# YuliangXiu/ICON

Measured on AMD Instinct MI355X. Metric: query-points/sec at 256^3 grid, higher is better.
Workload: dtype f32 via 3x f16 split MFMA (22-bit operands, f32 accumulate)

## Files before the change

icon_amd/csrc/fused_f16x3.hip:

```cpp
#pragma clang fp contract(off)

#include "geom_device.h"
#include "batch_device.h"
#include "mlp_f16x3_device.h"
#include "mlp_plain_device.h"
#include "sign_list_device.h"

#include <algorithm>
#include <mutex>

namespace icon {

constexpr int kTilePts = kF16Pts;
constexpr int kXsOff = kSideOff + 4352;
constexpr int kFusedLds = kXsOff + kTilePts * kXRow * 4;

struct FusedGeom {
    MeshDev m;
    FeatDev f;
    Calib cal;
    int res, z0;
    int off, nx, zs;
    const float *pts;
    int64_t N;
    const int *n_dev;
    const int32_t *out_map;
    float sdf_clip;
    int cmap_local;
    NearRef near;
    const uint8_t *code8;
    const int64_t *block_offsets;
    const unsigned long long *grp_mask;
    SignSrc sg;
    unsigned long long *clock;
    unsigned int *steal;
    int steal_static, steal_grp, steal_ngrp;
};
constexpr int kPoolOff = kSideOff + kSideFloats * 4;
enum { kPoolNext = 0, kPoolMask, kPoolDone, kPoolPer, kPoolRem, kPoolStatic, kPoolGroup, kPoolNGrp, kPoolGrid, kPoolWords };
static_assert(kPoolOff + 4 * kPoolWords <= kSideOff + 4352, "the draw state lives in the slack behind the side arrays");
constexpr int kPoolLenShift = 24;
constexpr int kMaxStealGroup = 127;

__device__ __forceinline__ void pool_draw(unsigned int *steal, volatile int *pool)
{
    unsigned xcc;
    asm volatile("s_getreg_b32 %0, hwreg(HW_REG_XCC_ID)" : "=s"(xcc));
    const int per = pool[kPoolPer], rem = pool[kPoolRem], stat = pool[kPoolStatic], grp = pool[kPoolGroup], ngrp = pool[kPoolNGrp],
              grid = pool[kPoolGrid];
    int mask = pool[kPoolMask], word = -1;
    for (int s = 0; s < 8 && word < 0; ++s) {
        const int x = (int)((xcc + (unsigned)s) & 7u);
        if ((mask >> x) & 1) continue;
        const int nwg = (grid - x + 7) >> 3;
        for (;;) {
            const int t = (int)atomicAdd(steal + x, 1u);
            if (t >= nwg * ngrp) { mask |= 1 << x; break; }
            const int k = t / ngrp, g = t - k * ngrp, b = x + 8 * k;
            const int sb = b * per + min(b, rem), eb = sb + per + (b < rem ? 1 : 0);
            const int a = sb + stat + g * grp;
            if (a < eb) { word = a | (min(grp, eb - a) << kPoolLenShift); break; }
        }
    }
    pool[kPoolMask] = mask;
    pool[kPoolNext] = word;
}

__device__ __forceinline__ void wg_stamp(unsigned long long *rec)
{
    rec[0] = __builtin_readcyclecounter();
    rec[1] = __builtin_amdgcn_s_memrealtime();
}

static_assert(kScanBlock == 256, "k_sign's 256-point blocks are the blocks of the outlier scan and the tiles of the fused kernel");
template <bool LATTICE>
// ... 73 lines not shown
        load_tri_full(m.tris + m.bin_slots[k], a, b, c, ia, ib, ic);
        cnt += ray_hit(p, a, b, c, ia, ib, ic);
    }
    cnt += __shfl_xor(cnt, 1);
    cnt += __shfl_xor(cnt, 2);
    if (live) {
        const bool ins = brute ? inside_brute(m, p) : ((cnt & 1) != 0);
        const bool far = box_dist2(d.box_lo[0], d.box_lo[1], d.box_lo[2], d.box_hi[0], d.box_hi[1], d.box_hi[2], p) > far_box2 || near_is_far(near, i);
        code = far ? sign_code_far(p, ins) : sign_code(p, near_d2(near, i), ins, sdf_clip);
        if (s == 0) code8[i] = (uint8_t)code;
    }
    unsigned long long x = __ballot(live && s == 0 && (code & kCodeOutlier));
    x = (x | (x >> 3)) & 0x0303030303030303ull;
    x = (x | (x >> 6)) & 0x000f000f000f000full;
    x = (x | (x >> 12)) & 0x000000ff000000ffull;
    x = (x | (x >> 24)) & 0xffffull;
    const int wave = threadIdx.x >> 6;
    if ((threadIdx.x & 63) == 0 && x) atomicOr(&gm[wave >> 2], x << (16 * (wave & 3)));
    __syncthreads();
    if (threadIdx.x < 4) grp_mask[(int64_t)blockIdx.x * 4 + threadIdx.x] = gm[threadIdx.x];
    if (threadIdx.x == 0) block_counts[blockIdx.x] = __popcll(gm[0]) + __popcll(gm[1]) + __popcll(gm[2]) + __popcll(gm[3]);
}

__global__ __launch_bounds__(256) void k_shell_zero(float *__restrict__ out, int res, int z0, int za, int zb, int row_wgs)
{
    const int planes = zb - za;
    if ((int)blockIdx.x < row_wgs) {
        const int64_t row = (int64_t)blockIdx.x * 256 + threadIdx.x;
        if (row >= (int64_t)planes * res) return;
        const int iy = (int)(row % res), iz = za + (int)(row / res);
        float *o = out + ((int64_t)(iz - z0) * res + iy) * res;
        o[0] = 0.0f; o[res - 1] = 0.0f;
        return;
    }
    const int f = ((int)blockIdx.x - row_wgs) * 4 + (int)(threadIdx.x >> 6);
    const int lane = threadIdx.x & 63;
    int iy, iz;
    if (f < 2 * planes) { iz = za + (f >> 1); iy = (f & 1) ? res - 1 : 0; }
    else {
        const int g = f - 2 * planes;
        const bool has0 = za == 0, has1 = zb == res;
        const int pl = g / res;
        if (pl >= (has0 ? 1 : 0) + (has1 ? 1 : 0)) return;
        iz = (pl == 0 && has0) ? 0 : res - 1;
        iy = g % res;
    }
    float *o = out + ((int64_t)(iz - z0) * res + iy) * res;
    for (int x = lane; x < res; x += 64) o[x] = 0.0f;
}

__device__ __forceinline__ int64_t lattice_item(const FusedGeom &G, int64_t q, int &ix, int &iy, int &iz)
{
    const uint32_t nx = (uint32_t)G.nx, qq = (uint32_t)q;
    const uint32_t r = qq / nx, lx = qq - r * nx, lz = r / nx, ly = r - lz * nx;
    ix = G.off + (int)lx; iy = G.off + (int)ly; iz = G.zs + (int)lz;
    return ((int64_t)(iz - G.z0) * G.res + iy) * G.res + ix;
}

__device__ __forceinline__ int64_t uniform64(int64_t v)
{
    const uint32_t lo = (uint32_t)__builtin_amdgcn_readfirstlane((int)(uint32_t)v);
    const uint32_t hi = (uint32_t)__builtin_amdgcn_readfirstlane((int)(uint32_t)((uint64_t)v >> 32));
    return (int64_t)(((uint64_t)hi << 32) | lo);
}

__device__ __forceinline__ void icon_row(const FusedGeom &G, const MeshDev &m, const FeatDev &f, f3 p, int64_t i, float *xrow, int64_t K, int64_t rank0)
{
    const uint32_t code = G.code8[i];
    Nearest nr;
    nr.slot = near_slot_of(G.near, i); nr.face = 0;
    nr.d2 = (code & kCodeOutlier) ? 0.0f : near_d2(G.near, i);
    const SdfOut o = sdf_attrs(m, p, nr, (code & kCodeInside) != 0);
    float s = o.sdf;
    f3 cmv = o.cm;
    if (code & kCodeOutlier) {
        s = (float)code_sign(code);
        if (G.cmap_local) cmv = mk3(s, s, s);
        else if (K > 0 && (f.smpl_mask & kSmplCmap)) {
            const int64_t blk = i >> 8;
            const int g = (int)(i >> 6) & 3;
            const unsigned long long *mk = G.grp_mask + blk * 4;
            int before = __popcll(mk[g] & ((1ull << (i & 63)) - 1ull));
            if (g > 0) before += __popcll(mk[0]);
            if (g > 1) before += __popcll(mk[1]);
            if (g > 2) before += __popcll(mk[2]);
            const int64_t jr = rank0 + G.block_offsets[blk] + before;
            float c3[3];
            outlier_cmap(G.sg, K, jr, c3);
            cmv = mk3(c3[0], c3[1], c3[2]);
        }
    }
    gather_planes_dyn(f, (f.n_select == 2 && o.vis == 0.0f) ? 1 : 0, p.x, p.y, xrow);
    int hh = f.csel;
    xrow[hh++] = s;
    if (f.smpl_mask & kSmplCmap) { xrow[hh] = cmv.x; xrow[hh + 1] = cmv.y; xrow[hh + 2] = cmv.z; hh += 3; }
    if (f.smpl_mask & kSmplNorm) { xrow[hh] = o.nrm.x; xrow[hh + 1] = o.nrm.y; xrow[hh + 2] = o.nrm.z; }
    xrow[kCodeSlot] = __int_as_float((int)(code & kCodeInCube));
}

template <int PRIOR, Src SRC>
__device__ __forceinline__ void build_row(const FusedGeom &G, const BatchDev &bd, int64_t q, float *xrow, int64_t K, int64_t rank0)
{
    f3 p;
    int64_t i;
    const int64_t b = SRC == Src::Batch ? q / bd.n : 0;
    if (SRC == Src::Lattice) {
        int ix, iy, iz;
// ... 40 lines not shown
    }

    issue_units(w.image, smem + kW0Off, kW0Bytes / 1024, wave0, lane0);
    float *side = reinterpret_cast<float *>(smem + kSideOff);
    for (int i = threadIdx.x; i < kSideFloats; i += kF16Block) side[i] = w.side[i];
    const float *sb0 = side, *sb1 = side + 512, *sb2 = side + 768, *sw3 = side + kW3Float;
    int64_t K = 0, rank0 = 0;
    if (PRIOR == ICON_PRIOR_ICON) launch_sign_extent(G, K, rank0);
    K = uniform64(K); rank0 = uniform64(rank0);

    if (SRC != Src::Batch && G.n_dev) { G.N = *G.n_dev; if (G.N <= 0) return; }
    const int tp = (SMALL && G.N <= (int64_t)(kTilePts / 2) * gridDim.x) ? kTilePts / 2 : kTilePts;
    const int ntiles = (int)((G.N + tp - 1) / tp);
    const bool stealing = !SMALL && G.steal != nullptr;
    const int per = ntiles / (int)gridDim.x, rem = ntiles % (int)gridDim.x;
    int tile = (int)blockIdx.x * per + min((int)blockIdx.x, rem);
    int tile_end = tile + (stealing ? min(G.steal_static, per) : per + ((int)blockIdx.x < rem ? 1 : 0));
    tile = __builtin_amdgcn_readfirstlane(tile);
    tile_end = __builtin_amdgcn_readfirstlane(tile_end);
    volatile int *pool = reinterpret_cast<volatile int *>(smem + kPoolOff);
    if (!SMALL) {
        if (threadIdx.x == 0) {
            pool[kPoolPer] = per; pool[kPoolRem] = rem; pool[kPoolStatic] = G.steal_static; pool[kPoolGroup] = G.steal_grp;
            pool[kPoolNGrp] = G.steal_ngrp; pool[kPoolGrid] = (int)gridDim.x; pool[kPoolDone] = 0; pool[kPoolMask] = 0; pool[kPoolNext] = -1;
            if (stealing && tile >= tile_end) pool_draw(G.steal, pool);
        }
        __syncthreads();
        if (stealing && tile >= tile_end) {
            const int word = __builtin_amdgcn_readfirstlane(pool[kPoolNext]);
            __syncthreads();
            if (word >= 0) { tile = word & ((1 << kPoolLenShift) - 1); tile_end = tile + (word >> kPoolLenShift); }
        }
    }
    if (tile < tile_end) issue_chunk(w.image, smem, 0, wave0, lane0);

    for (int nb = -1; tile < tile_end;) {
        int tid = threadIdx.x;
        asm volatile("" : "+v"(tid));
        const int lane = tid & 63, wave = __builtin_amdgcn_readfirstlane(tid >> 6);
        const int r = lane & 15, g = lane >> 4;
        const int t = tid;
        const bool draw = !SMALL && stealing && tile + 1 == tile_end;
        if (!SMALL && draw && t == 256) pool_draw(G.steal, pool);
        const bool worker = t < tp;
        int64_t q = (int64_t)tile * tp + (worker ? t : 0);
        if (q >= G.N) q = G.N - 1;
        if (worker) build_row<PRIOR, SRC>(G, bd, q, Xs + t * kXRow, K, rank0);
        __syncthreads();

        nb = (!SMALL && draw) ? __builtin_amdgcn_readfirstlane(pool[kPoolNext]) : -1;
        if (!SMALL && tid == 0) pool[kPoolDone] = pool[kPoolDone] + 1;
        const bool more = tile + 1 < tile_end || nb >= 0;
        if (SMALL && wave >= (tp >> 5)) {
            for (int c = 0; c < 16; ++c) {
                issue_chunk(w.image, smem + ((c + 1) & 1) * kBufBytes, c + 1, wave, lane);
                ICON_CHUNK_BARRIER();
            }
            issue_chunk(w.image, smem + kBufBytes, 17, wave, lane);
            ICON_CHUNK_BARRIER();
            issue_chunk(w.image, smem, 18, wave, lane);
            ICON_CHUNK_BARRIER();
            issue_chunk(w.image, smem + kBufBytes, 19, wave, lane);
            ICON_CHUNK_BARRIER();
            if (more) issue_chunk(w.image, smem, 0, wave, lane);
            ++tile;
            continue;
        }
        const int pt = wave * 32 + 16 * (g & 1) + r;
        half8 xb[2];
        const float tail = load_x(Xs + (wave * 32 + r) * kXRow + 8 * (g & 1), Xs + (wave * 32 + 16 + r) * kXRow + 8 * (g & 1), sw3, w.c0, g, xb);
        float maskf = (__float_as_int(Xs[pt * kXRow + kCodeSlot]) & (int)kCodeInCube) ? 1.0f : 0.0f;
        asm volatile("" : "+v"(maskf));

        f32x4 acc1[16][2];
#pragma unroll
        for (int m = 0; m < 16; ++m) acc1[m][0] = acc1[m][1] = *reinterpret_cast<const f32x4 *>(sb1 + m * 16 + 4 * g);
        half8 bh[2], bl[2];
        const LeakyK k0{w.inv0, w.p0, w.q0}, k1{w.inv1, w.p1, w.q1};
        {
            f32x4 h0[2][2];
            l0_tiles(smem + kW0Off, sb0, 0, xb, g, lane, h0);
            activate_split(h0[0][0], h0[0][1], h0[1][0], h0[1][1], k0, bh, bl);
        }
        f32x4 acc2[8][2];
        for (int c = 0; c < 15; ++c) {
            l01_chunk<false>(smem + (c & 1) * kBufBytes, smem + ((c + 1) & 1) * kBufBytes, smem + kW0Off, sb0, w.image, c, acc1, xb,
                             k0, g, lane, wave, bh, bl);
            ICON_CHUNK_BARRIER();
        }
        l01_chunk<true>(smem + kBufBytes, smem, smem + kW0Off, sb0, w.image, 15, acc1, xb, k0, g, lane, wave, bh, bl);
        ICON_CHUNK_BARRIER();
#pragma unroll
        for (int m2 = 0; m2 < 8; ++m2) acc2[m2][0] = acc2[m2][1] = *reinterpret_cast<const f32x4 *>(sb2 + m2 * 16 + 4 * g);
        activate_split(acc1[0][0], acc1[1][0], acc1[0][1], acc1[1][1], k1, bh, bl);
        l2_chunk<0>(smem, smem + kBufBytes, w.image, acc1, acc2, xb, k1, g, lane, wave, bh, bl);
        ICON_CHUNK_BARRIER();
        l2_chunk<1>(smem + kBufBytes, smem, w.image, acc1, acc2, xb, k1, g, lane, wave, bh, bl);
        ICON_CHUNK_BARRIER();
        l2_chunk<2>(smem, smem + kBufBytes, w.image, acc1, acc2, xb, k1, g, lane, wave, bh, bl);
        ICON_CHUNK_BARRIER();
        l2_chunk<3>(smem + kBufBytes, smem, w.image, acc1, acc2, xb, k1, g, lane, wave, bh, bl, more ? 0 : -1);

        float y2[2];
        {
            int tid_3 = threadIdx.x;
            asm volatile("" : "+v"(tid_3), "+v"(acc2[0][0]));
            l3_sum(sw3, acc2, tail, LeakyK{w.inv2, w.p2, w.q2}, w.b3, (tid_3 >> 4) & 3, y2);
        }
        int tid_o = threadIdx.x;
        asm volatile("" : "+v"(tid_o), "+v"(y2[0]), "+v"(y2[1]));
        const int g_o = (tid_o >> 4) & 3, pt_o = (tid_o >> 6) * 32 + 16 * (g_o & 1) + (tid_o & 15);
        const float y = apply_last_op(g_o == 0 ? y2[0] : y2[1], w.last_op);
        const int64_t oq = (int64_t)tile * tp + pt_o;
        if (g_o < 2 && oq < G.N) {
            int ix, iy, iz;
            out[SRC == Src::Lattice ? lattice_item(G, oq, ix, iy, iz) : ((SRC == Src::Points && G.out_map) ? (int64_t)G.out_map[oq] : oq)] = masked_result(y, maskf != 0.0f, w.flag);
        }
        if (!SMALL && nb >= 0) {
            tile = nb & ((1 << kPoolLenShift) - 1);
            tile_end = tile + (nb >> kPoolLenShift);
        } else ++tile;
    }
    if (!SMALL && stealing && threadIdx.x == 0) {
        __threadfence();
        if (atomicAdd(G.steal + 8, 1u) == gridDim.x - 1)
            for (int k = 0; k < 9; ++k) atomicExch(G.steal + k, 0u);
    }
    if (G.clock && threadIdx.x == 0 && blockIdx.x < kMaxProfGrid) {
        if (blockIdx.x == 0) wg_stamp(G.clock + 2);
        unsigned long long *rec = G.clock + 4 + kWgRec * blockIdx.x;
        wg_stamp(rec + 2);
        unsigned xcc, hw;
        asm volatile("s_getreg_b32 %0, hwreg(HW_REG_XCC_ID)" : "=s"(xcc));
        asm volatile("s_getreg_b32 %0, hwreg(HW_REG_HW_ID)" : "=s"(hw));
        rec[4] = ((unsigned long long)xcc << 32) | hw;
        rec[5] = SMALL ? 0ull : (unsigned long long)pool[kPoolDone];
    }
}

template <int PRIOR, Src SRC>
__global__ __launch_bounds__(64) void k_rescue_fused(FusedGeom G, float *__restrict__ out, MlpPlain P, const int *flag, int always, BatchDev bd)
{
    __shared__ float s[kPlainLds];
    if (!always && *flag == 0) return;
    if (SRC != Src::Batch && G.n_dev) G.N = *G.n_dev;
    const int lane = threadIdx.x;
    int64_t K = 0, rank0 = 0;
    if (PRIOR == ICON_PRIOR_ICON) launch_sign_extent(G, K, rank0);
    for (int64_t base = (int64_t)blockIdx.x * 64; base < G.N; base += (int64_t)gridDim.x * 64) {
        const int64_t q = base + lane;
        int ix, iy, iz;
        const int64_t o = q < G.N ? (SRC == Src::Lattice ? lattice_item(G, q, ix, iy, iz) : ((SRC == Src::Points && G.out_map) ? (int64_t)G.out_map[q] : q)) : 0;
        const float v = q < G.N ? out[o] : 0.0f;
        unsigned long long todo = __ballot(not_finite(v));
// ... 41 lines not shown
namespace {
constexpr int kMaxDevices = 64, kMaxKernelIds = 16;
std::mutex g_dev_mutex;
int g_n_cu[kMaxDevices];
bool g_attr_set[kMaxKernelIds][kMaxDevices];
}

int device_cu_count(int *n_cu)
{
    int dev = 0;
    ICON_HIP(hipGetDevice(&dev));
    ICON_ARG(dev >= 0 && dev < kMaxDevices, "device index out of range");
    std::lock_guard<std::mutex> lk(g_dev_mutex);
    if (!g_n_cu[dev]) {
        int n = 0;
        ICON_HIP(hipDeviceGetAttribute(&n, hipDeviceAttributeMultiprocessorCount, dev));
        g_n_cu[dev] = n > 0 ? n : 256;
    }
    *n_cu = g_n_cu[dev];
    return ICON_OK;
}

int once_per_device(int kernel_id, const std::function<hipError_t()> &set)
{
    int dev = 0;
    if (hipGetDevice(&dev) != hipSuccess || dev < 0 || dev >= kMaxDevices || kernel_id < 0 || kernel_id >= kMaxKernelIds) {
        const hipError_t e = set();
        return e == hipSuccess ? ICON_OK : fail(ICON_ERR_HIP, std::string("hipFuncSetAttribute: ") + hipGetErrorString(e));
    }
    std::lock_guard<std::mutex> lk(g_dev_mutex);
    if (g_attr_set[kernel_id][dev]) return ICON_OK;
    const hipError_t e = set();
    if (e != hipSuccess) return fail(ICON_ERR_HIP, std::string("hipFuncSetAttribute: ") + hipGetErrorString(e));
    g_attr_set[kernel_id][dev] = true;
    return ICON_OK;
}

int launch_fused_f16x3(const icon_mesh *mesh, const icon_feat *feat, const icon_mlp *mlp, int prior, const Calib &cal,
                       const LatticeMap &L, int za, int zb, const float *d_points, int64_t N, float sdf_clip, int cmap_local,
                       const icon_work *work, const SignSrc &fs, float *d_occ, bool lattice, hipStream_t st, const BatchDev *bd)
{
    FusedGeom G{};
    if (mesh) G.m = mesh->dev;
    G.f = feat->dev; G.cal = cal; G.pts = d_points; G.sdf_clip = sdf_clip; G.cmap_local = cmap_local;
    if (lattice) {
        const int zs = std::max(za, L.off), ze = std::min(zb, L.res - L.off);
        if (L.off) {
            const int64_t rows = (int64_t)(zb - za) * L.res;
            const int row_wgs = (int)((rows + 255) / 256);
            const int64_t face_rows = 2 * (int64_t)(zb - za) + (int64_t)((za == 0 ? 1 : 0) + (zb == L.res ? 1 : 0)) * L.res;
            if (rows > 0) hipLaunchKernelGGL(k_shell_zero, dim3((unsigned)(row_wgs + (face_rows + 3) / 4)), dim3(256), 0, st, d_occ, L.res, L.z0, za, zb, row_wgs);
        }
        G.res = L.res; G.z0 = L.z0; G.off = L.off; G.nx = L.res - 2 * L.off; G.zs = zs;
        N = (ze > zs) ? (int64_t)(ze - zs) * G.nx * G.nx : 0;
    }
    if (N <= 0) { ICON_HIP(hipGetLastError()); return ICON_OK; }
    ICON_ARG(N < (1ll << 31), "fused: more than 2^31 points in one call");
    G.N = N;
    G.near = work_near(work, mesh); G.code8 = work->d_code8;
    if (!lattice) { G.n_dev = work->q_n_dev; G.out_map = work->q_map; }
    G.clock = work->prof ? work->d_clock : nullptr;
    G.steal = nullptr; G.steal_static = 0; G.steal_grp = 1; G.steal_ngrp = 0;
    G.block_offsets = work->d_block_offsets; G.grp_mask = (const unsigned long long *)work->d_grp_mask;
    G.sg = fs;
    int rc = resolve_signs(work, &G.sg, st);
    if (rc) return rc;
    MlpF16Dev w;
    w.image = mlp->d_f16;
    w.side = reinterpret_cast<const float *>(mlp->d_f16 + kImageBytes);
    w.b3 = mlp->b3; w.inv0 = mlp->f16_inv[0]; w.inv1 = mlp->f16_inv[1]; w.inv2 = mlp->f16_inv[2]; w.c0 = mlp->c0; w.last_op = mlp->last_op;
    w.p0 = 0.505f * w.inv0; w.q0 = 0.495f * w.inv0; w.p1 = 0.505f * w.inv1; w.q1 = 0.495f * w.inv1; w.p2 = 0.505f * w.inv2; w.q2 = 0.495f * w.inv2;
    w.flag = work->d_flag ? work->d_flag : reinterpret_cast<int *>(mlp->d_blob + mlp->off_flag);
    const bool defer = work->defer_range_flag != nullptr;
    if (defer) w.flag = work->defer_range_flag;

    int n_cu = 0;
    if ((rc = device_cu_count(&n_cu))) return rc;
    if (defer) {}
    else if (work->d_flag) { if (!work->flag_clean) ICON_HIP(hipMemsetAsync(work->d_flag, 0, sizeof(int), st)); }
    else if ((rc = mlp_flag_reset(mlp, st))) return rc;
    work->flag_clean = false;
    const MlpPlain plain = mlp_plain_of(mlp);
    const int64_t n_resc = std::min<int64_t>((N + 63) / 64, 2048);
    const bool small = prior == ICON_PRIOR_ICON && (work->q_n_dev != nullptr || N <= 262144);
    const int64_t ntiles = small ? (N + kTilePts / 2 - 1) / (kTilePts / 2) : (N + kTilePts - 1) / kTilePts;
    const unsigned grid = (unsigned)std::min<int64_t>(ntiles, std::max(n_cu - work->reserve_cus, 1));
    {
        const int per = (int)(ntiles / grid);
        const int pool_len = (int)((int64_t)per * work->steal_permille / 1000);
        if (!small && !work->q_n_dev && work->d_steal && pool_len > 0 && ntiles > (int64_t)grid) {
            G.steal = work->d_steal; G.steal_grp = std::min(work->steal_grp, kMaxStealGroup);
            G.steal_static = per - pool_len;
            G.steal_ngrp = (pool_len + 1 + G.steal_grp - 1) / G.steal_grp;
        }
    }
    if (G.clock) work->clock_grid = (int)std::min<unsigned>(grid, (unsigned)kMaxProfGrid);
    const BatchDev batch = bd ? *bd : BatchDev{};
#define ICON_FUSED(P, S, ID, ...)                                                                                          \
    do {                                                                                                                   \
        if ((rc = once_per_device(ID, [] { return hipFuncSetAttribute(reinterpret_cast<const void *>(k_fused_f16x3<P, Src::S, ##__VA_ARGS__>), \
                                                                    hipFuncAttributeMaxDynamicSharedMemorySize, kFusedLds); }))) return rc; \
        hipLaunchKernelGGL((k_fused_f16x3<P, Src::S, ##__VA_ARGS__>), dim3(grid), dim3(kF16Block), kFusedLds, st, G, d_occ, w, batch); \
        debug_sync("k_fused_f16x3", st);                                                                                   \
        if (!defer) {                                                                                                      \
            hipLaunchKernelGGL((k_rescue_fused<P, Src::S>), dim3((unsigned)n_resc), dim3(64), 0, st, G, d_occ, plain, w.flag, rescue_always(), batch); \
            debug_sync("k_rescue_fused", st);                                                                              \
// ... 20 lines not shown
```

icon_amd/csrc/mlp_f16x3.hip:

```cpp
#include "mlp_f16x3_device.h"

#include <cmath>
#include <cstring>

namespace icon {

template <bool MASK>
__global__ __launch_bounds__(kF16Block, 2) void k_mlp_f16x3(const float *__restrict__ X, int64_t N, float *__restrict__ out, MlpF16Dev w)
{
    extern __shared__ __attribute__((aligned(16))) char smem[];
    const int lane = threadIdx.x & 63, wave = __builtin_amdgcn_readfirstlane(threadIdx.x >> 6);
    const int r = lane & 15, g = lane >> 4;
    const int64_t base = ((int64_t)blockIdx.x * (kF16Block / 64) + wave) * 32;
    const int64_t pi0 = min(base + r, N - 1), pi1 = min(base + 16 + r, N - 1);
    const int64_t po = (g & 1) ? pi1 : pi0;

    issue_units(w.image, smem + kW0Off, kW0Bytes / 1024, wave, lane);
    float *side = reinterpret_cast<float *>(smem + kSideOff);
    for (int i = threadIdx.x; i < kSideFloats; i += kF16Block) side[i] = w.side[i];
    const float *sb0 = side, *sb1 = side + 512, *sb2 = side + 768, *sw3 = side + kW3Float;

    float maskf = 1.0f;
    if (MASK) {
        const uint32_t code = (uint32_t)__float_as_int(X[po * kXRow + kCodeSlot]);
        maskf = (code & kCodeInCube) ? 1.0f : 0.0f;
        asm volatile("" : "+v"(maskf));
    }
    issue_chunk(w.image, smem, 0, wave, lane);
    __syncthreads();
    half8 xb[2];
    const float tail = load_x(X + pi0 * kXRow + 8 * (g & 1), X + pi1 * kXRow + 8 * (g & 1), sw3, w.c0, g, xb);

    f32x4 acc1[16][2];
#pragma unroll
    for (int m = 0; m < 16; ++m) acc1[m][0] = acc1[m][1] = *reinterpret_cast<const f32x4 *>(sb1 + m * 16 + 4 * g);

    half8 bh[2], bl[2];
    const LeakyK k0{w.inv0, w.p0, w.q0}, k1{w.inv1, w.p1, w.q1};
    {
        f32x4 h0[2][2];
        l0_tiles(smem + kW0Off, sb0, 0, xb, g, lane, h0);
        activate_split(h0[0][0], h0[0][1], h0[1][0], h0[1][1], k0, bh, bl);
    }
    for (int c = 0; c < 15; ++c) {
        l01_chunk<false>(smem + (c & 1) * kBufBytes, smem + ((c + 1) & 1) * kBufBytes, smem + kW0Off, sb0, w.image, c, acc1, xb,
                         k0, g, lane, wave, bh, bl);
        ICON_CHUNK_BARRIER();
    }
    l01_chunk<true>(smem + kBufBytes, smem, smem + kW0Off, sb0, w.image, 15, acc1, xb, k0, g, lane, wave, bh, bl);
    ICON_CHUNK_BARRIER();

    f32x4 acc2[8][2];
#pragma unroll
    for (int m2 = 0; m2 < 8; ++m2) acc2[m2][0] = acc2[m2][1] = *reinterpret_cast<const f32x4 *>(sb2 + m2 * 16 + 4 * g);
    activate_split(acc1[0][0], acc1[1][0], acc1[0][1], acc1[1][1], k1, bh, bl);
    l2_chunk<0>(smem, smem + kBufBytes, w.image, acc1, acc2, xb, k1, g, lane, wave, bh, bl);
    ICON_CHUNK_BARRIER();
    l2_chunk<1>(smem + kBufBytes, smem, w.image, acc1, acc2, xb, k1, g, lane, wave, bh, bl);
    ICON_CHUNK_BARRIER();
    l2_chunk<2>(smem, smem + kBufBytes, w.image, acc1, acc2, xb, k1, g, lane, wave, bh, bl);
    ICON_CHUNK_BARRIER();
    l2_chunk<3>(smem + kBufBytes, smem, w.image, acc1, acc2, xb, k1, g, lane, wave, bh, bl);

    float y2[2];
    {
        int tid_3 = threadIdx.x;
        asm volatile("" : "+v"(tid_3), "+v"(acc2[0][0]));
        l3_sum(sw3, acc2, tail, LeakyK{w.inv2, w.p2, w.q2}, w.b3, (tid_3 >> 4) & 3, y2);
    }
    int tid_o = threadIdx.x;
    asm volatile("" : "+v"(tid_o), "+v"(y2[0]), "+v"(y2[1]));
    const int g_o = (tid_o >> 4) & 3;
    const int64_t o = ((int64_t)blockIdx.x * (kF16Block / 64) + (tid_o >> 6)) * 32 + 16 * g_o + (tid_o & 15);
    const float y = apply_last_op(g_o == 0 ? y2[0] : y2[1], w.last_op);
    if (g_o < 2 && o < N) out[o] = masked_result(y, MASK ? maskf != 0.0f : true, w.flag);
}

uint16_t f32_to_f16_rtn(float f)
{
    uint32_t x; memcpy(&x, &f, 4);
    const uint32_t sign = (x >> 16) & 0x8000u;
    x &= 0x7fffffffu;
    if (x >= 0x7f800000u) return (uint16_t)(sign | 0x7c00u | (x > 0x7f800000u ? 0x200u : 0));
    if (x >= 0x477ff000u) return (uint16_t)(sign | 0x7c00u);
    if (x < 0x33000001u) return (uint16_t)sign;
    int e = (int)(x >> 23) - 127;
    uint32_t m = (x & 0x7fffffu) | 0x800000u;
    int shift;
    if (e < -14) { shift = 13 + (-14 - e); e = -15; } else shift = 13;
    uint32_t r = m >> shift;
    const uint32_t rem = m & ((1u << shift) - 1), half = 1u << (shift - 1);
    if (rem > half || (rem == half && (r & 1))) ++r;
    uint32_t out = (e == -15) ? r : (((uint32_t)(e + 15) << 10) + (r - 0x400u));
    return (uint16_t)(sign | out);
}

float f16_to_f32(uint16_t h)
{
    const uint32_t sign = (uint32_t)(h & 0x8000u) << 16;
    const int e = (h >> 10) & 31;
    const uint32_t m = h & 0x3ffu;
    float v;
    if (e == 0) v = std::ldexp((float)m, -24);
// ... 153 lines not shown
```

icon_amd/csrc/mlp_f16x3_device.h:

```cpp
#pragma once
#include "common.h"

namespace icon {

typedef float f32x4 __attribute__((ext_vector_type(4)));
typedef _Float16 half8 __attribute__((ext_vector_type(8)));
typedef __fp16 fp16x2 __attribute__((ext_vector_type(2)));
typedef __attribute__((address_space(1))) const void gvoid_t;
typedef __attribute__((address_space(3))) void lvoid_t;

constexpr int kF16Block = 512;
constexpr int kF16Pts = (kF16Block / 64) * 32;
constexpr int kBufBytes = 40 * 1024;
constexpr int kW3Stride = 40;
constexpr int kW3Float = 512 + 256 + 128;
constexpr int kZeroFloat = kW3Float + 4 * kW3Stride;
constexpr int kSideFloats = kZeroFloat + 4;
constexpr int kW0Off = 2 * kBufBytes;
constexpr int kW0Bytes = 32 * 1024;
constexpr int kSideOff = kW0Off + kW0Bytes;
constexpr int kLdsBytes = kSideOff + 4352;
constexpr int kZeroFromW0 = kSideOff + kZeroFloat * 4 - kW0Off;
constexpr int kZeroFromBuf0 = kSideOff + kZeroFloat * 4;
static_assert(kSideFloats * 4 <= 4352 && kZeroFromW0 % 16 == 0, "side arrays");
// ... 9 lines not shown
    float inv0, inv1, inv2;
    float p0, q0, p1, q1, p2, q2;
    int c0;
    int last_op;
    int *flag;
};

__device__ __forceinline__ float masked_result(float y, bool in_cube, int *flag)
{
    if (in_cube && not_finite(y)) *flag = 1;
    return in_cube ? y : 0.0f;
}

__device__ __forceinline__ fp16x2 residual_pair(fp16x2 hh, float v0, float v1)
{
    const int hb = __builtin_bit_cast(int, hh);
    int lb;
    asm("v_fma_mixlo_f16 %0, %1, -1.0, %2 op_sel_hi:[1,0,0]" : "=v"(lb) : "v"(hb), "v"(v0));
    asm("v_fma_mixhi_f16 %0, %1, -1.0, %2 op_sel:[1,0,0] op_sel_hi:[1,0,0]" : "+v"(lb) : "v"(hb), "v"(v1));
    return __builtin_bit_cast(fp16x2, lb);
}

__device__ __forceinline__ void split8(const float *v, half8 &hi, half8 &lo)
{
#pragma unroll
    for (int q = 0; q < 4; ++q) {
        const fp16x2 h = __builtin_amdgcn_cvt_pkrtz(v[2 * q], v[2 * q + 1]);
        const fp16x2 l = residual_pair(h, v[2 * q], v[2 * q + 1]);
        hi[2 * q] = (_Float16)h[0]; hi[2 * q + 1] = (_Float16)h[1];
        lo[2 * q] = (_Float16)l[0]; lo[2 * q + 1] = (_Float16)l[1];
    }
}

#ifndef ICON_ACT_EXACT
#define ICON_ACT_EXACT 0
#endif
struct LeakyK { float inv, p, q; };
__device__ __forceinline__ float leaky_scaled(float a, const LeakyK &k)
{
#if ICON_ACT_EXACT
    const float x = a * k.inv;
    return fmaxf(x, 0.01f * x);
#else
    return fmaf(fabsf(a), k.q, k.p * a);
#endif
}

#define MFMA32(a, b, c) __builtin_amdgcn_mfma_f32_16x16x32_f16((a), (b), (c), 0, 0, 0)

__device__ __forceinline__ half8 lds_op(const char *buf, int slot, int lane)
{
    return *reinterpret_cast<const half8 *>(buf + slot * 1024 + lane * 16);
}

#define ICON_CHUNK_BARRIER() __syncthreads()


__device__ __forceinline__ void issue_units(const char *src, char *buf, int units, int wave, int lane)
{
    for (int u = wave; u < units; u += kF16Block / 64)
        __builtin_amdgcn_global_load_lds((gvoid_t *)(src + u * 1024 + lane * 16), (lvoid_t *)(buf + u * 1024), 16, 0, 0);
}
__device__ __forceinline__ void issue_chunk(const char *image, char *buf, int k, int wave, int lane)
{
    issue_units(image + (size_t)chunk_offset(k) * 1024, buf, chunk_units(k), wave, lane);
}


#define GROUP6(ACC, M, AH, AL, BH, BL)                                                              \
    ACC[M][0] = MFMA32(AH, BH[0], ACC[M][0]); ACC[M][1] = MFMA32(AH, BH[1], ACC[M][1]);             \
    ACC[M][0] = MFMA32(AH, BL[0], ACC[M][0]); ACC[M][1] = MFMA32(AH, BL[1], ACC[M][1]);             \
    ACC[M][0] = MFMA32(AL, BH[0], ACC[M][0]); ACC[M][1] = MFMA32(AL, BH[1], ACC[M][1]);

__device__ __forceinline__ float load_x(const float *row0, const float *row1, const float *__restrict__ sw3, int c0, int g, half8 (&xb)[2])
{
    float tail = 0.0f;
#pragma unroll
    for (int b = 0; b < 2; ++b) {
        const float4 *q = reinterpret_cast<const float4 *>(b ? row1 : row0);
        const float4 u = q[0], v = q[1];
        float x[8] = {u.x, u.y, u.z, u.w, v.x, v.y, v.z, v.w};
#pragma unroll
        for (int s = 0; s < 8; ++s) x[s] = (s + 8 * (g & 1) < c0) ? x[s] : 0.0f;
        half8 hi, lo;
        split8(x, hi, lo);
        xb[b] = g < 2 ? hi : lo;
        float t = 0.0f;
#pragma unroll
        for (int s = 0; s < 8; ++s) t = fmaf(sw3[g * kW3Stride + 32 + s], x[s], t);
        tail = (g >> 1) == b ? t : tail;
    }
    asm volatile("" : "+v"(tail));
    return tail;
}

__device__ __forceinline__ void raw_operands(const char *__restrict__ base, int tile, int zero_off, int g, int lane, half8 &a1, half8 &a2)
{
    const int col = (lane & 31) * 16;
    const int lo_off = g < 2 ? 512 + col : zero_off, lo_mul = g < 2 ? 1024 : 0;
    a1 = *reinterpret_cast<const half8 *>(base + tile * 1024 + col);
    a2 = *reinterpret_cast<const half8 *>(base + lo_off + tile * lo_mul);
}

__device__ __forceinline__ void l0_tiles(const char *__restrict__ W0, const float *__restrict__ sb0, int c, const half8 (&xb)[2],
                                         int g, int lane, f32x4 (&h0)[2][2])
{
#pragma unroll
    for (int t = 0; t < 2; ++t) {
        const f32x4 bias = *reinterpret_cast<const f32x4 *>(sb0 + (2 * c + t) * 16 + 4 * g);
        half8 a1, a2;
        raw_operands(W0, 2 * c + t, kZeroFromW0, g, lane, a1, a2);
        h0[0][t] = MFMA32(a1, xb[0], bias); h0[1][t] = MFMA32(a1, xb[1], bias);
        h0[0][t] = MFMA32(a2, xb[0], h0[0][t]); h0[1][t] = MFMA32(a2, xb[1], h0[1][t]);
    }
}

__device__ __forceinline__ void act_part(const f32x4 &ta0, const f32x4 &tb0, const f32x4 &ta1, const f32x4 &tb1, int k, const LeakyK &inv,
                                         half8 (&nh)[2], half8 (&nl)[2])
{
    const int b = k >> 2, q = k & 3, j0 = (q & 1) * 2;
    const f32x4 &src = b ? (q >> 1 ? tb1 : ta1) : (q >> 1 ? tb0 : ta0);
    const float v0 = leaky_scaled(src[j0], inv), v1 = leaky_scaled(src[j0 + 1], inv);
    fp16x2 hh = __builtin_amdgcn_cvt_pkrtz(v0, v1);
    fp16x2 ll = residual_pair(hh, v0, v1);
    int hb = __builtin_bit_cast(int, hh), lb = __builtin_bit_cast(int, ll);
    asm volatile("" : "+v"(hb), "+v"(lb));
    hh = __builtin_bit_cast(fp16x2, hb); ll = __builtin_bit_cast(fp16x2, lb);
    nh[b][2 * q] = (_Float16)hh[0]; nh[b][2 * q + 1] = (_Float16)hh[1];
    nl[b][2 * q] = (_Float16)ll[0]; nl[b][2 * q + 1] = (_Float16)ll[1];
}

__device__ __forceinline__ void activate_split(const f32x4 &ta0, const f32x4 &tb0, const f32x4 &ta1, const f32x4 &tb1, const LeakyK &inv,
                                               half8 (&bh)[2], half8 (&bl)[2])
{
#pragma unroll
    for (int k = 0; k < 8; ++k) act_part(ta0, tb0, ta1, tb1, k, inv, bh, bl);
}

template <bool LAST>
__device__ __forceinline__ void l01_chunk(const char *__restrict__ L, char *__restrict__ nxt, const char *__restrict__ W0,
                                          const float *__restrict__ sb0, const char *image, int c, f32x4 (&acc1)[16][2],
                                          const half8 (&xb)[2], const LeakyK &inv0, int g4, int lane, int wave,
                                          half8 (&bh)[2], half8 (&bl)[2])
{
    issue_chunk(image, nxt, c + 1, wave, lane);
    f32x4 h0n[2][2];
    if (!LAST) l0_tiles(W0, sb0, c + 1, xb, g4, lane, h0n);
    half8 nh[2], nl[2];
    half8 a[2][2];
    a[0][0] = lds_op(L, 0, lane); a[0][1] = lds_op(L, 1, lane);
    __builtin_amdgcn_sched_barrier(0);
#pragma unroll
    for (int t = 0; t < 16; ++t) {
        if (t + 1 < 16) { a[(t + 1) & 1][0] = lds_op(L, 2 * t + 2, lane); a[(t + 1) & 1][1] = lds_op(L, 2 * t + 3, lane); }
        GROUP6(acc1, t, a[t & 1][0], a[t & 1][1], bh, bl)
        if (!LAST && (t & 1)) act_part(h0n[0][0], h0n[0][1], h0n[1][0], h0n[1][1], t >> 1, inv0, nh, nl);
        __builtin_amdgcn_sched_barrier(0);
    }
    if (!LAST) { bh[0] = nh[0]; bh[1] = nh[1]; bl[0] = nl[0]; bl[1] = nl[1]; }
}

template <int Q>
__device__ __forceinline__ void l2_chunk(const char *__restrict__ L, char *__restrict__ nxt, const char *image,
                                         f32x4 (&acc1)[16][2], f32x4 (&acc2)[8][2], const half8 (&xb)[2], const LeakyK &inv1,
                                         int g4, int lane, int wave, half8 (&bh)[2], half8 (&bl)[2], int next_chunk = (Q < 3) ? 17 + Q : -1)
{
    if (next_chunk >= 0) issue_chunk(image, nxt, next_chunk, wave, lane);
    if (Q == 0) {
#pragma unroll
        for (int m2 = 0; m2 < 8; ++m2) {
            half8 a1, a2;
            raw_operands(L, 32 + m2, kZeroFromBuf0, g4, lane, a1, a2);
            acc2[m2][0] = MFMA32(a1, xb[0], acc2[m2][0]); acc2[m2][1] = MFMA32(a1, xb[1], acc2[m2][1]);
            acc2[m2][0] = MFMA32(a2, xb[0], acc2[m2][0]); acc2[m2][1] = MFMA32(a2, xb[1], acc2[m2][1]);
        }
        __builtin_amdgcn_sched_barrier(0);
    }
#pragma unroll
    for (int mm = 0; mm < 2; ++mm) {
        constexpr int kLast = 7;
        const int kk = 2 * Q + mm, n = kk < kLast ? 2 * kk + 2 : 0;
        half8 nh[2], nl[2];
        half8 a[2][2];
        a[0][0] = lds_op(L, mm * 16, lane); a[0][1] = lds_op(L, mm * 16 + 1, lane);
        __builtin_amdgcn_sched_barrier(0);
#pragma unroll
        for (int t = 0; t < 8; ++t) {
            if (t + 1 < 8) { a[(t + 1) & 1][0] = lds_op(L, mm * 16 + 2 * t + 2, lane); a[(t + 1) & 1][1] = lds_op(L, mm * 16 + 2 * t + 3, lane); }
            GROUP6(acc2, t, a[t & 1][0], a[t & 1][1], bh, bl)
            if (kk < kLast) act_part(acc1[n][0], acc1[n + 1][0], acc1[n][1], acc1[n + 1][1], t, inv1, nh, nl);
            __builtin_amdgcn_sched_barrier(0);
        }
        if (kk < kLast) { bh[0] = nh[0]; bh[1] = nh[1]; bl[0] = nl[0]; bl[1] = nl[1]; }
    }
}

__device__ __forceinline__ void l3_sum(const float *__restrict__ sw3, const f32x4 (&acc2)[8][2], float tail, const LeakyK &inv2,
                                       float b3, int g, float (&y)[2])
{
    const float *w3 = sw3 + g * kW3Stride;
    float part[2] = {0.0f, 0.0f};
#pragma unroll
    for (int m2 = 0; m2 < 8; ++m2) {
        const f32x4 wv = *reinterpret_cast<const f32x4 *>(w3 + 4 * m2);
#pragma unroll
        for (int j = 0; j < 4; ++j) {
            part[0] = fmaf(wv[j], leaky_scaled(acc2[m2][0][j], inv2), part[0]);
            part[1] = fmaf(wv[j], leaky_scaled(acc2[m2][1][j], inv2), part[1]);
        }
    }
    const float t = tail + __shfl_xor(tail, 16);
    const float t_other = __shfl_xor(t, 32);
#pragma unroll
    for (int b = 0; b < 2; ++b) {
        part[b] += __shfl_xor(part[b], 16);
        part[b] += __shfl_xor(part[b], 32);
        y[b] = (part[b] + ((g >> 1) == b ? t : t_other)) + b3;
    }
}

// ... 2 lines not shown
```

Baseline: 1.109 billion.

## Specialize chunk prefetch loops with compile-time unit counts and LDS address-space pointers

Replaces the generic per-chunk loader with templated compile-time unit counts and streams layer-0/1 chunks through a pair-unrolled, nounroll loop whose weight, bias and chunk pointers advance incrementally as LDS address-space pointers instead of being recomputed from chunk indices. Lattice index decoding uses a precomputed magic-number division instead of hardware-less integer divides. The aim is to cut scalar and vector address arithmetic and loop overhead around the MFMA pipeline. It hardcodes per-chunk unit counts (32, and 40 for the last chunk), which ties the code to the current weight image layout.

```diff
diff --git a/icon_amd/csrc/fused_f16x3.hip b/icon_amd/csrc/fused_f16x3.hip
--- a/icon_amd/csrc/fused_f16x3.hip
+++ b/icon_amd/csrc/fused_f16x3.hip
@@ -21,6 +21,7 @@
     Calib cal;
     int res, z0;
     int off, nx, zs;
+    uint32_t nx_magic;
     const float *pts;
     int64_t N;
     const int *n_dev;
@@ -200,7 +201,7 @@
 __device__ __forceinline__ int64_t lattice_item(const FusedGeom &G, int64_t q, int &ix, int &iy, int &iz)
 {
     const uint32_t nx = (uint32_t)G.nx, qq = (uint32_t)q;
-    const uint32_t r = qq / nx, lx = qq - r * nx, lz = r / nx, ly = r - lz * nx;
+    const uint32_t r = udiv_fast(qq, nx, G.nx_magic), lx = qq - r * nx, lz = udiv_fast(r, nx, G.nx_magic), ly = r - lz * nx;
     ix = G.off + (int)lx; iy = G.off + (int)ly; iz = G.zs + (int)lz;
     return ((int64_t)(iz - G.z0) * G.res + iy) * G.res + ix;
 }
@@ -347,17 +348,24 @@
         if (!SMALL && tid == 0) pool[kPoolDone] = pool[kPoolDone] + 1;
         const bool more = tile + 1 < tile_end || nb >= 0;
         if (SMALL && wave >= (tp >> 5)) {
-            for (int c = 0; c < 16; ++c) {
-                issue_chunk(w.image, smem + ((c + 1) & 1) * kBufBytes, c + 1, wave, lane);
+#pragma nounroll
+            for (int c = 0; c < 14; c += 2) {
+                issue_chunk_units<32>(w.image, smem + kBufBytes, c + 1, wave, lane);
+                ICON_CHUNK_BARRIER();
+                issue_chunk_units<32>(w.image, smem, c + 2, wave, lane);
                 ICON_CHUNK_BARRIER();
             }
-            issue_chunk(w.image, smem + kBufBytes, 17, wave, lane);
+            issue_chunk_units<32>(w.image, smem + kBufBytes, 15, wave, lane);
             ICON_CHUNK_BARRIER();
-            issue_chunk(w.image, smem, 18, wave, lane);
+            issue_chunk_units<40>(w.image, smem, 16, wave, lane);
             ICON_CHUNK_BARRIER();
-            issue_chunk(w.image, smem + kBufBytes, 19, wave, lane);
+            issue_chunk_units<32>(w.image, smem + kBufBytes, 17, wave, lane);
             ICON_CHUNK_BARRIER();
-            if (more) issue_chunk(w.image, smem, 0, wave, lane);
+            issue_chunk_units<32>(w.image, smem, 18, wave, lane);
+            ICON_CHUNK_BARRIER();
+            issue_chunk_units<32>(w.image, smem + kBufBytes, 19, wave, lane);
+            ICON_CHUNK_BARRIER();
+            if (more) issue_chunk_units<32>(w.image, smem, 0, wave, lane);
             ++tile;
             continue;
         }
@@ -372,19 +380,8 @@
         for (int m = 0; m < 16; ++m) acc1[m][0] = acc1[m][1] = *reinterpret_cast<const f32x4 *>(sb1 + m * 16 + 4 * g);
         half8 bh[2], bl[2];
         const LeakyK k0{w.inv0, w.p0, w.q0}, k1{w.inv1, w.p1, w.q1};
-        {
-            f32x4 h0[2][2];
-            l0_tiles(smem + kW0Off, sb0, 0, xb, g, lane, h0);
-            activate_split(h0[0][0], h0[0][1], h0[1][0], h0[1][1], k0, bh, bl);
-        }
         f32x4 acc2[8][2];
-        for (int c = 0; c < 15; ++c) {
-            l01_chunk<false>(smem + (c & 1) * kBufBytes, smem + ((c + 1) & 1) * kBufBytes, smem + kW0Off, sb0, w.image, c, acc1, xb,
-                             k0, g, lane, wave, bh, bl);
-            ICON_CHUNK_BARRIER();
-        }
-        l01_chunk<true>(smem + kBufBytes, smem, smem + kW0Off, sb0, w.image, 15, acc1, xb, k0, g, lane, wave, bh, bl);
-        ICON_CHUNK_BARRIER();
+        layer01(smem, sb0, w.image, acc1, xb, k0, g, lane, wave, bh, bl);
 #pragma unroll
         for (int m2 = 0; m2 < 8; ++m2) acc2[m2][0] = acc2[m2][1] = *reinterpret_cast<const f32x4 *>(sb2 + m2 * 16 + 4 * g);
         activate_split(acc1[0][0], acc1[1][0], acc1[0][1], acc1[1][1], k1, bh, bl);
@@ -394,7 +391,7 @@
         ICON_CHUNK_BARRIER();
         l2_chunk<2>(smem, smem + kBufBytes, w.image, acc1, acc2, xb, k1, g, lane, wave, bh, bl);
         ICON_CHUNK_BARRIER();
-        l2_chunk<3>(smem + kBufBytes, smem, w.image, acc1, acc2, xb, k1, g, lane, wave, bh, bl, more ? 0 : -1);
+        l2_chunk<3>(smem + kBufBytes, smem, w.image, acc1, acc2, xb, k1, g, lane, wave, bh, bl, more);
 
         float y2[2];
         {
@@ -542,6 +539,7 @@
             if (rows > 0) hipLaunchKernelGGL(k_shell_zero, dim3((unsigned)(row_wgs + (face_rows + 3) / 4)), dim3(256), 0, st, d_occ, L.res, L.z0, za, zb, row_wgs);
         }
         G.res = L.res; G.z0 = L.z0; G.off = L.off; G.nx = L.res - 2 * L.off; G.zs = zs;
+        G.nx_magic = udiv_magic((uint32_t)std::max(G.nx, 1));
         N = (ze > zs) ? (int64_t)(ze - zs) * G.nx * G.nx : 0;
     }
     if (N <= 0) { ICON_HIP(hipGetLastError()); return ICON_OK; }
diff --git a/icon_amd/csrc/mlp_f16x3.hip b/icon_amd/csrc/mlp_f16x3.hip
--- a/icon_amd/csrc/mlp_f16x3.hip
+++ b/icon_amd/csrc/mlp_f16x3.hip
@@ -37,18 +37,7 @@
 
     half8 bh[2], bl[2];
     const LeakyK k0{w.inv0, w.p0, w.q0}, k1{w.inv1, w.p1, w.q1};
-    {
-        f32x4 h0[2][2];
-        l0_tiles(smem + kW0Off, sb0, 0, xb, g, lane, h0);
-        activate_split(h0[0][0], h0[0][1], h0[1][0], h0[1][1], k0, bh, bl);
-    }
-    for (int c = 0; c < 15; ++c) {
-        l01_chunk<false>(smem + (c & 1) * kBufBytes, smem + ((c + 1) & 1) * kBufBytes, smem + kW0Off, sb0, w.image, c, acc1, xb,
-                         k0, g, lane, wave, bh, bl);
-        ICON_CHUNK_BARRIER();
-    }
-    l01_chunk<true>(smem + kBufBytes, smem, smem + kW0Off, sb0, w.image, 15, acc1, xb, k0, g, lane, wave, bh, bl);
-    ICON_CHUNK_BARRIER();
+    layer01(smem, sb0, w.image, acc1, xb, k0, g, lane, wave, bh, bl);
 
     f32x4 acc2[8][2];
 #pragma unroll
diff --git a/icon_amd/csrc/mlp_f16x3_device.h b/icon_amd/csrc/mlp_f16x3_device.h
--- a/icon_amd/csrc/mlp_f16x3_device.h
+++ b/icon_amd/csrc/mlp_f16x3_device.h
@@ -85,6 +85,15 @@
 {
     return *reinterpret_cast<const half8 *>(buf + slot * 1024 + lane * 16);
 }
+typedef __attribute__((address_space(3))) const char *lds_cptr;
+typedef __attribute__((address_space(3))) const half8 *lds_half8;
+typedef __attribute__((address_space(3))) const f32x4 *lds_f32x4;
+__device__ __forceinline__ lds_cptr lds_lane_address(const void *p)
+{
+    unsigned a = (unsigned)(size_t)(__attribute__((address_space(3))) const void *)p;
+    asm("" : "+v"(a));
+    return (lds_cptr)(size_t)a;
+}
 
 #define ICON_CHUNK_BARRIER() __syncthreads()
 
@@ -97,6 +106,25 @@
 __device__ __forceinline__ void issue_chunk(const char *image, char *buf, int k, int wave, int lane)
 {
     issue_units(image + (size_t)chunk_offset(k) * 1024, buf, chunk_units(k), wave, lane);
+}
+template <int UNITS>
+__device__ __forceinline__ void issue_wave_units(const char *src, char *dst, unsigned &lane_off)
+{
+    constexpr int kWaves = kF16Block / 64;
+    static_assert(UNITS % kWaves == 0, "every wave issues the same number of pieces");
+    asm volatile("" : "+v"(lane_off));
+#pragma unroll
+    for (int j = 0; j < UNITS / kWaves; ++j) {
+        const char *piece = src + j * kWaves * 1024;
+        asm volatile("" : "+s"(piece));
+        __builtin_amdgcn_global_load_lds((gvoid_t *)(piece + lane_off), (lvoid_t *)(dst + j * kWaves * 1024), 16, 0, 0);
+    }
+}
+template <int UNITS>
+__device__ __forceinline__ void issue_chunk_units(const char *image, char *buf, int k, int wave, int lane)
+{
+    unsigned lane_off = (unsigned)lane * 16u;
+    issue_wave_units<UNITS>(image + (size_t)(chunk_offset(k) + wave) * 1024, buf + wave * 1024, lane_off);
 }
 
 
@@ -135,15 +163,23 @@
     a2 = *reinterpret_cast<const half8 *>(base + lo_off + tile * lo_mul);
 }
 
-__device__ __forceinline__ void l0_tiles(const char *__restrict__ W0, const float *__restrict__ sb0, int c, const half8 (&xb)[2],
-                                         int g, int lane, f32x4 (&h0)[2][2])
+struct L0At { lds_cptr hi, lo, bias; int lo_step; };
+__device__ __forceinline__ L0At l0_begin(const char *W0, const float *sb0, int g, int lane)
+{
+    const int col = (lane & 31) * 16;
+    return L0At{lds_lane_address(W0 + col), lds_lane_address(W0 + (g < 2 ? 512 + col : kZeroFromW0)), lds_lane_address(sb0 + 4 * g), g < 2 ? 1024 : 0};
+}
+
+template <int K>
+__device__ __forceinline__ void l0_tiles(lds_cptr __restrict__ hi, lds_cptr __restrict__ lo, int lo_step, lds_cptr __restrict__ bias,
+                                         const half8 (&xb)[2], f32x4 (&h0)[2][2])
 {
 #pragma unroll
     for (int t = 0; t < 2; ++t) {
-        const f32x4 bias = *reinterpret_cast<const f32x4 *>(sb0 + (2 * c + t) * 16 + 4 * g);
-        half8 a1, a2;
-        raw_operands(W0, 2 * c + t, kZeroFromW0, g, lane, a1, a2);
-        h0[0][t] = MFMA32(a1, xb[0], bias); h0[1][t] = MFMA32(a1, xb[1], bias);
+        const f32x4 b = *(lds_f32x4)(bias + (K + t) * 64);
+        const half8 a1 = *(lds_half8)(hi + (K + t) * 1024);
+        const half8 a2 = *(lds_half8)(lo + t * lo_step);
+        h0[0][t] = MFMA32(a1, xb[0], b); h0[1][t] = MFMA32(a1, xb[1], b);
         h0[0][t] = MFMA32(a2, xb[0], h0[0][t]); h0[1][t] = MFMA32(a2, xb[1], h0[1][t]);
     }
 }
@@ -170,35 +206,65 @@
     for (int k = 0; k < 8; ++k) act_part(ta0, tb0, ta1, tb1, k, inv, bh, bl);
 }
 
-template <bool LAST>
-__device__ __forceinline__ void l01_chunk(const char *__restrict__ L, char *__restrict__ nxt, const char *__restrict__ W0,
-                                          const float *__restrict__ sb0, const char *image, int c, f32x4 (&acc1)[16][2],
-                                          const half8 (&xb)[2], const LeakyK &inv0, int g4, int lane, int wave,
-                                          half8 (&bh)[2], half8 (&bl)[2])
-{
-    issue_chunk(image, nxt, c + 1, wave, lane);
+template <bool LAST, int K0>
+__device__ __forceinline__ void l01_chunk(lds_cptr __restrict__ L, char *__restrict__ nxt, lds_cptr __restrict__ w_hi,
+                                          lds_cptr __restrict__ w_lo, int lo_step, lds_cptr __restrict__ bias, const char *next_src,
+                                          f32x4 (&acc1)[16][2], const half8 (&xb)[2], const LeakyK &inv0, unsigned &lane_off, int wave,
+                                          const half8 (&bh)[2], const half8 (&bl)[2], half8 (&nh)[2], half8 (&nl)[2])
+{
+    issue_wave_units<LAST ? 40 : 32>(next_src, nxt + wave * 1024, lane_off);
     f32x4 h0n[2][2];
-    if (!LAST) l0_tiles(W0, sb0, c + 1, xb, g4, lane, h0n);
-    half8 nh[2], nl[2];
+    if (!LAST) l0_tiles<K0>(w_hi, w_lo, lo_step, bias, xb, h0n);
     half8 a[2][2];
-    a[0][0] = lds_op(L, 0, lane); a[0][1] = lds_op(L, 1, lane);
+    a[0][0] = *(lds_half8)L; a[0][1] = *(lds_half8)(L + 1024);
     __builtin_amdgcn_sched_barrier(0);
 #pragma unroll
     for (int t = 0; t < 16; ++t) {
-        if (t + 1 < 16) { a[(t + 1) & 1][0] = lds_op(L, 2 * t + 2, lane); a[(t + 1) & 1][1] = lds_op(L, 2 * t + 3, lane); }
+        if (t + 1 < 16) { a[(t + 1) & 1][0] = *(lds_half8)(L + (2 * t + 2) * 1024); a[(t + 1) & 1][1] = *(lds_half8)(L + (2 * t + 3) * 1024); }
         GROUP6(acc1, t, a[t & 1][0], a[t & 1][1], bh, bl)
         if (!LAST && (t & 1)) act_part(h0n[0][0], h0n[0][1], h0n[1][0], h0n[1][1], t >> 1, inv0, nh, nl);
         __builtin_amdgcn_sched_barrier(0);
     }
-    if (!LAST) { bh[0] = nh[0]; bh[1] = nh[1]; bl[0] = nl[0]; bl[1] = nl[1]; }
+}
+
+__device__ __forceinline__ void layer01(char *smem, const float *sb0, const char *image, f32x4 (&acc1)[16][2], const half8 (&xb)[2],
+                                        const LeakyK &inv0, int g, int lane, int wave, half8 (&bh)[2], half8 (&bl)[2])
+{
+    char *const buf0 = smem, *const buf1 = smem + kBufBytes;
+    const lds_cptr col0 = lds_lane_address(buf0 + lane * 16), col1 = lds_lane_address(buf1 + lane * 16);
+    unsigned lane_off = (unsigned)lane * 16u;
+    L0At at = l0_begin(smem + kW0Off, sb0, g, lane);
+    {
+        f32x4 h0[2][2];
+        l0_tiles<0>(at.hi, at.lo, at.lo_step, at.bias, xb, h0);
+        activate_split(h0[0][0], h0[0][1], h0[1][0], h0[1][1], inv0, bh, bl);
+    }
+    at.lo += 2 * at.lo_step;
+    const char *src = image + (size_t)(chunk_offset(1) + wave) * 1024;
+    half8 nh[2], nl[2];
+#pragma nounroll
+    for (int p = 0; p < 7; ++p) {
+        l01_chunk<false, 2>(col0, buf1, at.hi, at.lo, at.lo_step, at.bias, src, acc1, xb, inv0, lane_off, wave, bh, bl, nh, nl);
+        at.lo += 2 * at.lo_step;
+        ICON_CHUNK_BARRIER();
+        l01_chunk<false, 4>(col1, buf0, at.hi, at.lo, at.lo_step, at.bias, src + 32 * 1024, acc1, xb, inv0, lane_off, wave, nh, nl, bh, bl);
+        at.lo += 2 * at.lo_step;
+        ICON_CHUNK_BARRIER();
+        at.hi += 4 * 1024; at.bias += 4 * 64;
+        src += 64 * 1024;
+    }
+    l01_chunk<false, 2>(col0, buf1, at.hi, at.lo, at.lo_step, at.bias, src, acc1, xb, inv0, lane_off, wave, bh, bl, nh, nl);
+    ICON_CHUNK_BARRIER();
+    l01_chunk<true, 0>(col1, buf0, at.hi, at.lo, at.lo_step, at.bias, src + 32 * 1024, acc1, xb, inv0, lane_off, wave, nh, nl, bh, bl);
+    ICON_CHUNK_BARRIER();
 }
 
 template <int Q>
 __device__ __forceinline__ void l2_chunk(const char *__restrict__ L, char *__restrict__ nxt, const char *image,
                                          f32x4 (&acc1)[16][2], f32x4 (&acc2)[8][2], const half8 (&xb)[2], const LeakyK &inv1,
-                                         int g4, int lane, int wave, half8 (&bh)[2], half8 (&bl)[2], int next_chunk = (Q < 3) ? 17 + Q : -1)
-{
-    if (next_chunk >= 0) issue_chunk(image, nxt, next_chunk, wave, lane);
+                                         int g4, int lane, int wave, half8 (&bh)[2], half8 (&bl)[2], bool issue_next = Q < 3)
+{
+    if (issue_next) issue_chunk_units<32>(image, nxt, Q < 3 ? 17 + Q : 0, wave, lane);
     if (Q == 0) {
 #pragma unroll
         for (int m2 = 0; m2 < 8; ++m2) {
```

Result: faster. 1.128 billion (median of 6 runs) (+1.7%).
